# SimonMacLean/NeRF-or-nothing

Measured on AMD Instinct MI355X. Metric: train rays/sec (128 samples/ray, 8×256 MLP) at 1/2/4/8 MI355X; PSNR vs ref, higher is better.
Workload: dtype f32; 1 GPU; BASELINE configs[1]: 1024-ray global batch x 128+128 samples, 8x256 MLP fwd/bwd + Adam; global_batch=1024, rays_per_gpu=1024, micro_batch=1024, parallelism=dp1, precision=f32

## Files before the change

### nerf-or-nothing_amd/csrc/kernels/mlp16.h

```cpp
#pragma once
#include "mlp_common.h"

namespace nof {

constexpr int kMlp16Threads = 512;
constexpr int kIpe16Floats = 6 * 64 * 4;

__device__ __forceinline__ f32x4 mfma16(float a, float b, f32x4 c) {
  return __builtin_amdgcn_mfma_f32_16x16x4f32(a, b, c, 0, 0, 0);
}

__device__ __forceinline__ void slice16_dma_step(const float* __restrict__ src, float* dst, int tid, int i) {
  const int wave = tid >> 6;
  const __amdgpu_buffer_rsrc_t rsrc =
      __builtin_amdgcn_make_buffer_rsrc(const_cast<float*>(src), (short)0, 0x7fffffff, 0x00020000);
  __builtin_amdgcn_raw_ptr_buffer_load_lds(rsrc, (lptr_t)(dst + (kMlp16Threads * i + 64 * wave) * 4), 16, tid * 16,
                                           i * kMlp16Threads * 16, 0, 0);
}
__device__ __forceinline__ void slice16_dma(const float* __restrict__ src, float* dst, int tid) {
#pragma unroll
  for (int i = 0; i < 4; ++i) slice16_dma_step(src, dst, tid, i);
}

template <int P> constexpr int ring16_slots() { return P == 0 ? 4 : 3; }
template <int P> constexpr int ring16_floats() { return ring16_slots<P>() * kSliceFloats; }
__device__ __forceinline__ void ring16_prologue(const float* __restrict__ img, float* lds, int tid) {
  slice16_dma(img, lds, tid);
  slice16_dma(img + kSliceFloats, lds + kSliceFloats, tid);
}

__device__ __forceinline__ constexpr int feat16(int t, int g, int r) { return 16 * t + 4 * g + r; }

constexpr int kStoreNT = 2;
struct BlkStore16 {
  static constexpr bool kHalf = false;
  uint32_t voff[4];
  __device__ __forceinline__ BlkStore16(int lane, int half) {
    const int g = lane >> 4, s = 16 * half + (lane & 15);
#pragma unroll
    for (int r = 0; r < 4; ++r)
      voff[r] = 512u * g + ((((s >> 2) ^ (4 * (g & 1) + r)) << 4) | ((s & 3) << 2));
  }
  __device__ __forceinline__ void store(__amdgpu_buffer_rsrc_t blk, int t, int r, float v) const {
    __builtin_amdgcn_raw_buffer_store_b32(__float_as_uint(v), blk, (int)voff[r], 2048 * t + 128 * r, kStoreNT);
  }
};
__device__ __forceinline__ __amdgpu_buffer_rsrc_t blk_rsrc(float* blk) {
  return __builtin_amdgcn_make_buffer_rsrc(blk, (short)0, 0x7fffffff, 0x00020000);
}

template <bool kNT>
struct BlkStore16H {
  static constexpr bool kHalf = true;
  uint32_t voff;
  uint32_t voff2;
  uint32_t sel;
  __device__ __forceinline__ BlkStore16H(int lane, int half) {
    const int g = lane >> 4, j = lane & 15;
    voff = 256u * g + ((((2 * half + (j >> 3)) ^ g) << 4) | ((j & 7) << 1));
    voff2 = 256u * g + 64u * (j & 1) + ((((2 * half + (j >> 3)) ^ g) << 4) | ((j & 6) << 1));
    sel = (j & 1) ? 0x03020706u : 0x05040100u;
  }
  __device__ __forceinline__ void store_pairs(__amdgpu_buffer_rsrc_t blk, int t, uint32_t p01, uint32_t p23) const {
    const uint32_t q01 = (uint32_t)__builtin_amdgcn_mov_dpp((int)p01, 0xB1, 0xF, 0xF, false);
    const uint32_t q23 = (uint32_t)__builtin_amdgcn_mov_dpp((int)p23, 0xB1, 0xF, 0xF, false);
    __builtin_amdgcn_raw_buffer_store_b32(__builtin_amdgcn_perm(q01, p01, sel), blk, (int)voff2, 1024 * t,
                                          kNT ? kStoreNT : 0);
    __builtin_amdgcn_raw_buffer_store_b32(__builtin_amdgcn_perm(q23, p23, sel), blk, (int)voff2 + 128, 1024 * t,
                                          kNT ? kStoreNT : 0);
  }
  __device__ __forceinline__ void store(__amdgpu_buffer_rsrc_t blk, int t, int r, float v) const {
    store_h(blk, t, r, (_Float16)v);
  }
  __device__ __forceinline__ void store_h(__amdgpu_buffer_rsrc_t blk, int t, int r, _Float16 h) const {
    __builtin_amdgcn_raw_buffer_store_b16(__builtin_bit_cast(unsigned short, h), blk, (int)voff + 64 * r, 1024 * t,
                                          kNT ? kStoreNT : 0);
  }
};
template <int P, bool kBwd> struct Store16 { typedef BlkStore16 T; typedef float E; };
template <bool kBwd> struct Store16<2, kBwd> { typedef BlkStore16H<true> T; typedef _Float16 E; };
template <class E>
// ... 26 lines not shown
  typedef float f2 __attribute__((ext_vector_type(2)));
  hi01 = __builtin_bit_cast(uint32_t, __builtin_convertvector((f2{x[0], x[1]}), h2));
  hi23 = __builtin_bit_cast(uint32_t, __builtin_convertvector((f2{x[2], x[3]}), h2));
  float r[4];
  asm("v_fma_mix_f32 %0, %1, 1.0, -%2 op_sel_hi:[0,0,1]" : "=v"(r[0]) : "v"(x[0]), "v"(hi01));
  asm("v_fma_mix_f32 %0, %1, 1.0, -%2 op_sel:[0,0,1] op_sel_hi:[0,0,1]" : "=v"(r[1]) : "v"(x[1]), "v"(hi01));
  asm("v_fma_mix_f32 %0, %1, 1.0, -%2 op_sel_hi:[0,0,1]" : "=v"(r[2]) : "v"(x[2]), "v"(hi23));
  asm("v_fma_mix_f32 %0, %1, 1.0, -%2 op_sel:[0,0,1] op_sel_hi:[0,0,1]" : "=v"(r[3]) : "v"(x[3]), "v"(hi23));
  lo01 = __builtin_bit_cast(uint32_t, __builtin_convertvector((f2{r[0], r[1]}), h2));
  lo23 = __builtin_bit_cast(uint32_t, __builtin_convertvector((f2{r[2], r[3]}), h2));
}

template <bool kSplit, bool kStore, class ST>
__device__ __forceinline__ void put_tile(float (&bin)[16][4], int t, const float (&v)[4], const ST& bst,
                                         __amdgpu_buffer_rsrc_t blk) {
  if constexpr (kSplit) {
    uint32_t hi01, hi23, lo01, lo23;
    split4h(v, hi01, hi23, lo01, lo23);
    const int row = t & ~1, c = 2 * (t & 1);
    bin[row][c] = __uint_as_float(hi01);
    bin[row][c + 1] = __uint_as_float(hi23);
    bin[row + 1][c] = __uint_as_float(lo01);
    bin[row + 1][c + 1] = __uint_as_float(lo23);
    if constexpr (kStore) {
      if constexpr (ST::kHalf) {
        bst.store_pairs(blk, t, hi01, hi23);
      } else {
#pragma unroll
        for (int r = 0; r < 4; ++r) bst.store(blk, t, r, v[r]);
      }
    }
  } else {
#pragma unroll
    for (int r = 0; r < 4; ++r) {
      bin[t][r] = v[r];
      if constexpr (kStore) bst.store(blk, t, r, v[r]);
    }
  }
}

struct NoEpi16 {
  static constexpr int kVmPerPart = 0;
  __device__ __forceinline__ void operator()(int) {}
};

template <int NT_B, int NT_I, int OT, int kSlots, class Epi>
__device__ __forceinline__ void mlp_layer16(const float (&bin)[16][4], const float* ipe, f32x4 (&acc)[16],
                                            float* lds, int& cur, const float*& wsrc, bool last_in_schedule, int tid,
                                            int lane, Epi& epi, const float* cinit) {
  static_assert(OT % 2 == 0 && OT <= 16, "row tiles come in pairs");
  constexpr int NG = OT;
  constexpr int kEpiGroup1 = 4;
  constexpr int kEpiGroup2 = (NG / 2 + 4 < NG) ? NG / 2 + 4 : NG - 1;
  const int g = lane >> 4;
  const int row = lane & 15;
  const int swz = (row >> 1) & 7;
#pragma unroll
  for (int t = 0; t < NT_B + NT_I; ++t) {
    const bool dma = !(last_in_schedule && t + 2 >= NT_B + NT_I);
    const int nxt2 = kSlots == 4 ? ((cur + 2) & 3) : (cur == 0 ? 2 : cur - 1);
    const float* W = lds + cur * kSliceFloats + row * 32;
    auto aread = [&](int q, int which) {
      const int tt = q / (OT / 2), p = q % (OT / 2);
      return *reinterpret_cast<const f32x4*>(W + (2 * p + which) * 16 * 32 + (((4 * tt + g) ^ swz) << 2));
    };
    f32x4 a0 = aread(0, 0), a1 = aread(0, 1);
    auto cread = [&](int p, int which) { return *reinterpret_cast<const f32x4*>(cinit + 16 * (2 * p + which)); };
    f32x4 c0 = {}, c1 = {};
    if (t == 0 && cinit) { c0 = cread(0, 0); c1 = cread(0, 1); }
#pragma unroll
    for (int q = 0; q < NG; ++q) {
      const int tt = q / (OT / 2), p = q % (OT / 2);
      f32x4 b4;
      if (t < NT_B) {
        const int tb = (t < NT_B) ? 2 * t + tt : 0;
        b4[0] = bin[tb][0]; b4[1] = bin[tb][1]; b4[2] = bin[tb][2]; b4[3] = bin[tb][3];
      } else {
        const int ti = (t >= NT_B) ? 2 * (t - NT_B) + tt : 0;
        if constexpr (kSlots == 4) {
          b4[0] = ipe[4 * ti]; b4[1] = ipe[4 * ti + 1]; b4[2] = ipe[4 * ti + 2]; b4[3] = ipe[4 * ti + 3];
        } else b4 = *reinterpret_cast<const f32x4*>(ipe + (ti * 64 + lane) * 4);
      }
      asm volatile("" ::"v"(a0), "v"(a1), "v"(c0), "v"(c1));
      f32x4 n0 = a0, n1 = a1, m0 = c0, m1 = c1;
      if (q + 1 < NG) {
        n0 = aread(q + 1, 0);
        n1 = aread(q + 1, 1);
      }
      if (t == 0 && cinit && q + 1 < OT / 2) { m0 = cread(q + 1, 0); m1 = cread(q + 1, 1); }
      if (dma && q < 4) slice16_dma_step(wsrc + 2 * kSliceFloats, lds + nxt2 * kSliceFloats, tid, q);
      __builtin_amdgcn_sched_barrier(0);
      const bool first = t == 0 && tt == 0;
#pragma unroll
      for (int r = 0; r < 4; ++r) {
        acc[2 * p] = mfma16(a0[r], b4[r], (first && r == 0) ? c0 : acc[2 * p]);
        acc[2 * p + 1] = mfma16(a1[r], b4[r], (first && r == 0) ? c1 : acc[2 * p + 1]);
      }
      if (t + 1 < NT_B && q == kEpiGroup1) epi(2 * t + 2);
      if (t + 1 < NT_B && q == kEpiGroup2) epi(2 * t + 3);
      __builtin_amdgcn_sched_barrier(0);
      a0 = n0;
      a1 = n1;
      c0 = m0;
      c1 = m1;
    }
    if constexpr (kSlots == 4) {
      if (cur & 1) slice_barrier(t + 1 < NT_B ? 2 * Epi::kVmPerPart : 0);
      cur = (cur + 1) & 3;
    } else {
      slice_barrier((dma ? 4 : 0) + (t + 1 < NT_B ? 2 * Epi::kVmPerPart : 0));
      cur = cur == 2 ? 0 : cur + 1;
    }
    wsrc += kSliceFloats;
  }
}
template <int NT_B, int NT_I, int OT, class Epi>
__device__ __forceinline__ void mlp_layer16h(const float (&bin)[16][4], const float* ipe_lds, f32x4 (&acc)[16],
                                             float* lds, int& cur, const float*& wsrc, bool last_in_schedule, int tid,
                                             int lane, Epi& epi, const float* cinit) {
  typedef SplitMode<2> SM;
  static_assert(OT % 2 == 0 && OT <= 16, "row tiles come in pairs");
  constexpr int kPieces = 2;
  constexpr int kPP0 = 0;
  constexpr int kDmaSteps = 4;
  constexpr int kSlots = ring16_slots<2>();
  constexpr int NG = OT / 2;
  constexpr int kE1 = NG > 4 ? 4 : NG - 1;
  constexpr int kE2 = NG > 6 ? 6 : NG - 1;
#pragma unroll
  for (int t = 0; t < NT_B + NT_I; ++t) {
    const bool dma = !(last_in_schedule && t + 2 >= NT_B + NT_I);
    const int nxt2 = kSlots == 4 ? ((cur + 2) & 3) : (cur == 0 ? 2 : cur - 1);
    const f16x8* W = reinterpret_cast<const f16x8*>(lds + cur * kSliceFloats) + lane;
    Frag<2> b;
    float v[8];
    if (t < NT_B) {
      const int tb = t < NT_B ? 2 * t : 0;
      const f32x4 hi = {bin[tb][0], bin[tb][1], bin[tb][2], bin[tb][3]};
      const f32x4 lo = {bin[tb + 1][0], bin[tb + 1][1], bin[tb + 1][2], bin[tb + 1][3]};
      b.p[0] = __builtin_bit_cast(f16x8, hi);
      b.p[1] = __builtin_bit_cast(f16x8, lo);
    } else {
      const int ti = t >= NT_B ? 2 * (t - NT_B) : 0;
      if constexpr (kSlots == 4) {
#pragma unroll
        for (int i = 0; i < 8; ++i) v[i] = ipe_lds[4 * ti + i];
      } else {
        const f32x4 u0 = *reinterpret_cast<const f32x4*>(ipe_lds + (ti * 64 + lane) * 4);
        const f32x4 u1 = *reinterpret_cast<const f32x4*>(ipe_lds + ((ti + 1) * 64 + lane) * 4);
#pragma unroll
        for (int i = 0; i < 4; ++i) { v[i] = u0[i]; v[4 + i] = u1[i]; }
      }
      split8<2>(v, b);
    }
    Frag<2> a0, a1;
#pragma unroll
    for (int p = 0; p < kPieces; ++p) { a0.p[p] = W[(16 * p) * 64]; a1.p[p] = W[(16 * p + 1) * 64]; }
    auto cread = [&](int rt) { return *reinterpret_cast<const f32x4*>(cinit + 16 * rt); };
    f32x4 c0 = {}, c1 = {};
    if (t == 0 && cinit) { c0 = cread(0); c1 = cread(1); }
#pragma unroll
    for (int q = 0; q < NG; ++q) {
      if constexpr (kPieces == 2) asm volatile("" ::"v"(a0.p[0]), "v"(a0.p[1]), "v"(a1.p[0]), "v"(a1.p[1]), "v"(c0), "v"(c1));
      else asm volatile("" ::"v"(a0.p[0]), "v"(a1.p[0]), "v"(c0), "v"(c1));
      Frag<2> n0 = a0, n1 = a1;
      f32x4 m0 = c0, m1 = c1;
      if (t == 0 && cinit && q + 1 < NG) { m0 = cread(2 * q + 2); m1 = cread(2 * q + 3); }
      if (q + 1 < NG) {
#pragma unroll
        for (int p = 0; p < kPieces; ++p) {
          n0.p[p] = W[(16 * p + 2 * q + 2) * 64];
          n1.p[p] = W[(16 * p + 2 * q + 3) * 64];
        }
      }
      if (dma && q < kDmaSteps) slice16_dma_step(wsrc + 2 * kSliceFloats, lds + nxt2 * kSliceFloats, tid, q);
      __builtin_amdgcn_sched_barrier(0);
      const bool first = t == 0;
#pragma unroll
      for (int pp = kPP0; pp < SM::NPROD; ++pp) {
        acc[2 * q] = SM::mfma16(a0.p[SM::pa(pp)], b.p[SM::pb(pp)], (first && pp == kPP0) ? c0 : acc[2 * q]);
        acc[2 * q + 1] = SM::mfma16(a1.p[SM::pa(pp)], b.p[SM::pb(pp)], (first && pp == kPP0) ? c1 : acc[2 * q + 1]);
      }
      if (t + 1 < NT_B && q == kE1) epi(2 * t + 2);
      if (t + 1 < NT_B && q == kE2) epi(2 * t + 3);
      __builtin_amdgcn_sched_barrier(0);
      a0 = n0;
      a1 = n1;
      c0 = m0;
      c1 = m1;
    }
    if constexpr (kSlots == 4) {
      if (cur & 1) slice_barrier(t + 1 < NT_B ? 2 * Epi::kVmPerPart : 0);
      cur = (cur + 1) & 3;
    } else {
      slice_barrier((dma ? kDmaSteps : 0) + (t + 1 < NT_B ? 2 * Epi::kVmPerPart : 0));
      cur = cur == 2 ? 0 : cur + 1;
    }
    wsrc += kSliceFloats;
  }
}

template <int P, int NT_B, int NT_I, int OT, class Epi>
__device__ __forceinline__ void layer16(const float (&bin)[16][4], const float* ipe_lds, f32x4 (&acc)[16], float* lds,
                                        int& cur, const float*& wsrc, bool last_in_schedule, int tid, int lane,
                                        Epi& epi, const float* cinit = nullptr) {
  if constexpr (P == 2 || P == 3)
    mlp_layer16h<NT_B, NT_I, OT>(bin, ipe_lds, acc, lds, cur, wsrc, last_in_schedule, tid, lane, epi, cinit);
  else
    mlp_layer16<NT_B, NT_I, OT, ring16_slots<P>()>(bin, ipe_lds, acc, lds, cur, wsrc, last_in_schedule, tid, lane,
                                                   epi, cinit);
}
template <int P, int NT_B, int NT_I, int OT>
__device__ __forceinline__ void layer16(const float (&bin)[16][4], const float* ipe_lds, f32x4 (&acc)[16], float* lds,
                                        int& cur, const float*& wsrc, bool last_in_schedule, int tid, int lane,
                                        const float* cinit = nullptr) {
  NoEpi16 none;
  layer16<P, NT_B, NT_I, OT>(bin, ipe_lds, acc, lds, cur, wsrc, last_in_schedule, tid, lane, none, cinit);
}

}
```

### nerf-or-nothing_amd/csrc/kernels/mlp_bwd16.hip

```cpp
#include "common.h"
#include "launch.h"
#include "mlp16.h"

namespace nof {


template <bool kDensity, class ST, bool kSplit = false>
struct BwdEpi16 {
  static constexpr int kVmPerPart = 4;
  const f32x4 (&acc)[16];
  float (&bin)[16][4];
  const ST& bst;
  const int g;
  const float* w8;
  float dzs;
  __amdgpu_buffer_rsrc_t dst_blk;
  uint2 mk;
  f32x4 wnext;

  __device__ __forceinline__ BwdEpi16(const f32x4 (&acc_)[16], float (&bin_)[16][4], const ST& bst_, int lane)
      : acc(acc_), bin(bin_), bst(bst_), g(lane >> 4) {}
  template <class E>
  __device__ __forceinline__ void begin(const uint2* mask, E* dst_blk_, const float* w8_ = nullptr, float dzs_ = 0.0f) {
    mk = *mask;
    dst_blk = blk_rsrc_t(dst_blk_);
    if constexpr (kDensity) {
      w8 = w8_ + 4 * g;
      dzs = dzs_;
      wnext = *reinterpret_cast<const f32x4*>(w8);
    }
  }
  __device__ __forceinline__ void operator()(int t) {
    f32x4 w4;
    if constexpr (kDensity) {
      w4 = wnext;
      if (t + 1 < 16) wnext = *reinterpret_cast<const f32x4*>(w8 + 16 * (t + 1));
    }
    float v[4];
#pragma unroll
    for (int r = 0; r < 4; ++r) {
      v[r] = acc[t][r];
      if constexpr (kDensity) v[r] = __builtin_fmaf(w4[r], dzs, v[r]);
      v[r] = mask16_apply(mk, t, r, v[r]);
    }
    put_tile<kSplit, true>(bin, t, v, bst, dst_blk);
  }
  __device__ __forceinline__ void tile01() {
    (*this)(0);
    (*this)(1);
  }
};

template <int P>
__global__ __launch_bounds__(kMlp16Threads, 1) void k_mlp_bwd16(BwdArgs a) {
  typedef typename Store16<P, true>::T ST;
  typedef typename Store16<P, true>::E AE;
  __shared__ __attribute__((aligned(16))) float lds[ring16_floats<P>() + 256];
  float* w8_lds = lds + ring16_floats<P>();
  const int tid = threadIdx.x, lane = tid & 63, g = lane >> 4, j = lane & 15;
  const int wave = __builtin_amdgcn_readfirstlane(tid >> 6);
  const int half = wave & 1;
  const ST bst(lane, half);
  const int nblk = a.M / kBlk;
  const int blk_raw = blockIdx.x * 4 + (wave >> 1);
  const int blk = blk_raw < nblk ? blk_raw : nblk - 1;
  const int m = blk * kBlk + 16 * half + j;
  NOF_DCHECK(a.M % kBlk == 0 && blk >= 0 && blk < nblk, kChkMlpBlock);
  const float* tail = a.wimg_b + (size_t)kBwdSlices * kSliceFloats;
  const size_t layer_stride = (size_t)nblk * kWidth * kBlk;
  uint32_t* masks = const_cast<uint32_t*>(a.masks);

  ring16_prologue(a.wimg_b, lds, tid);

  const f32x4 zh = reinterpret_cast<const f32x4*>(a.zhead)[m];
  float dzs = a.dsigma[m] * sigmoid_f(zh[0] + a.dbias);
  float dzc[3];
#pragma unroll
  for (int c = 0; c < 3; ++c) {
    const float s = sigmoid_f(zh[1 + c]);
    dzc[c] = a.drgb[(size_t)m * 3 + c] * (s * (1.0f - s)) * a.rgb_scale;
  }
  if constexpr (P >= 2) {
    const float sc = delta_scale(a.amax, false);
    dzs *= sc;
#pragma unroll
    for (int c = 0; c < 3; ++c) dzc[c] *= sc;
  }
  const __amdgpu_buffer_rsrc_t d9 = blk_rsrc_t(reinterpret_cast<AE*>(a.delta9x) + (size_t)blk * kD9F * kBlk);
#pragma unroll
  for (int r = 0; r < 4; ++r) bst.store(d9, 8, r, g == 0 ? (r == 0 ? dzs : dzc[r - 1]) : 0.0f);
  float bin[16][4];
  {
    const uint2 mk = *mask16_ptr(masks, blk, 8, half, lane);
    const float* w10 = tail + kBwdTailW10;
#pragma unroll
    for (int t = 0; t < 8; ++t) {
      const int fb = 16 * t + 4 * g;
      const f32x4 wa = *reinterpret_cast<const f32x4*>(w10 + fb);
      const f32x4 wb = *reinterpret_cast<const f32x4*>(w10 + 128 + fb);
      const f32x4 wc = *reinterpret_cast<const f32x4*>(w10 + 256 + fb);
      float v[4];
#pragma unroll
      for (int r = 0; r < 4; ++r)
        v[r] = mask16_apply(mk, t, r, __builtin_fmaf(wc[r], dzc[2], __builtin_fmaf(wb[r], dzc[1], wa[r] * dzc[0])));
      put_tile<P >= 2, true>(bin, t, v, bst, d9);
    }
  }
  if (tid < 64) reinterpret_cast<f32x4*>(w8_lds)[tid] = reinterpret_cast<const f32x4*>(tail + kBwdTailW8)[tid];
  __syncthreads();

  int cur = 0;
  const float* wsrc = a.wimg_b;
  f32x4 accA[16], accB[16];
  AE* delta_blk = reinterpret_cast<AE*>(a.delta) + (size_t)blk * kWidth * kBlk;
  BwdEpi16<true, ST, P >= 2> e7(accA, bin, bst, lane);
  e7.begin(mask16_ptr(masks, blk, 7, half, lane), delta_blk + 7 * layer_stride, w8_lds, dzs);
  layer16<P, 4, 0, 16>(bin, nullptr, accA, lds, cur, wsrc, false, tid, lane);
  e7.tile01();
  BwdEpi16<false, ST, P >= 2> ea(accA, bin, bst, lane), eb(accB, bin, bst, lane);
  eb.begin(mask16_ptr(masks, blk, 6, half, lane), delta_blk + 6 * layer_stride);
  layer16<P, 8, 0, 16>(bin, nullptr, accB, lds, cur, wsrc, false, tid, lane, e7);
  eb.tile01();
  static_assert(kDepth == 8, "bwd pairing assumes 8 trunk layers");
  for (int l = kDepth - 2; l >= 2; l -= 2) {
    ea.begin(mask16_ptr(masks, blk, l - 1, half, lane), delta_blk + (l - 1) * layer_stride);
    layer16<P, 8, 0, 16>(bin, nullptr, accA, lds, cur, wsrc, false, tid, lane, eb);
    ea.tile01();
    eb.begin(mask16_ptr(masks, blk, l - 2, half, lane), delta_blk + (l - 2) * layer_stride);
    layer16<P, 8, 0, 16>(bin, nullptr, accB, lds, cur, wsrc, l == 2, tid, lane, ea);
    eb.tile01();
  }
#pragma unroll
  for (int t = 2; t < 16; ++t) eb(t);
}

hipError_t launch_mlp_bwd16(const BwdArgs& a, hipStream_t st) {
  const int nblk = a.M / kBlk;
  if (a.split == 2) hipLaunchKernelGGL(k_mlp_bwd16<2>, dim3((nblk + 3) / 4), dim3(kMlp16Threads), 0, st, a);
  else if (a.split == 3) hipLaunchKernelGGL(k_mlp_bwd16<3>, dim3((nblk + 3) / 4), dim3(kMlp16Threads), 0, st, a);
  else hipLaunchKernelGGL(k_mlp_bwd16<0>, dim3((nblk + 3) / 4), dim3(kMlp16Threads), 0, st, a);
  return hipGetLastError();
}

NOF_CHECK_UNIT(check_unit_mlp_bwd16)

}
```

### nerf-or-nothing_amd/csrc/kernels/mlp_fwd16.hip

```cpp
#include "common.h"
#include "geometry.h"
#include "launch.h"
#include "mlp16.h"

namespace nof {


template <bool store, bool kDensity, int NT, class ST, bool kSplit = false>
struct FwdEpi16 {
  static constexpr int kVmPerPart = store ? 4 : 0;
  const f32x4 (&acc)[16];
  float (&bin)[16][4];
  const ST& bst;
  const int g;
  const float* w8;
  __amdgpu_buffer_rsrc_t act_blk;
  uint2* mask_dst;
  uint32_t mw[2];
  f32x4 wnext;
  float zs;

  __device__ __forceinline__ FwdEpi16(const f32x4 (&acc_)[16], float (&bin_)[16][4], const ST& bst_, int lane)
      : acc(acc_), bin(bin_), bst(bst_), g(lane >> 4) {}
  template <class E>
  __device__ __forceinline__ void begin(E* act_blk_, uint2* mask_dst_, const float* w8_ = nullptr) {
    act_blk = blk_rsrc_t(act_blk_);
    mask_dst = mask_dst_;
    mw[0] = mw[1] = 0u;
    if constexpr (kDensity) {
      w8 = w8_ + 4 * g;
      wnext = *reinterpret_cast<const f32x4*>(w8);
      zs = 0.0f;
    }
  }
  __device__ __forceinline__ void operator()(int t) {
    const bool more = t + 1 < NT;
    f32x4 w4;
    if constexpr (kDensity) {
      w4 = wnext;
      if (more) wnext = *reinterpret_cast<const f32x4*>(w8 + 16 * (t + 1));
    }
    float hv[4];
#pragma unroll
    for (int r = 0; r < 4; ++r) {
      hv[r] = relu_bit(acc[t][r], mw[t >> 3]);
      if constexpr (kDensity) zs = __builtin_fmaf(w4[r], hv[r], zs);
    }
    put_tile<kSplit, store>(bin, t, hv, bst, act_blk);
    if constexpr (store && kVmPerPart > 0)
      if (!more) *mask_dst = make_uint2(mw[0], mw[1]);
  }
  __device__ __forceinline__ void tile01() {
    (*this)(0);
    (*this)(1);
  }
};

template <int P, bool store>
__global__ __launch_bounds__(kMlp16Threads, 1) void k_mlp_fwd16(FwdArgs a) {
  typedef typename Store16<P, false>::T ST;
  typedef typename Store16<P, false>::E AE;
  constexpr int kRing = ring16_slots<P>() * kSliceFloats;
  constexpr bool kIpeReg = ring16_slots<P>() == 4;
  constexpr int kIpeLds = kIpeReg ? 0 : 8 * kIpe16Floats;
  constexpr int kBiasLds = 8 * 256 + 256;
  __shared__ __attribute__((aligned(16))) float lds[kRing + kIpeLds + 8 * 128 + kBiasLds];
  const int tid = threadIdx.x, lane = tid & 63, g = lane >> 4, j = lane & 15;
  const int wave = __builtin_amdgcn_readfirstlane(tid >> 6);
  const int half = wave & 1;
  const int nblk = a.M / kBlk;
  const int blk_raw = blockIdx.x * 4 + (wave >> 1);
  const int blk = blk_raw < nblk ? blk_raw : nblk - 1;
  const int m0 = blk * kBlk;
  const int ray = m0 / a.S;
  const int s0 = m0 - ray * a.S + 16 * half;
  const int m = m0 + 16 * half + j;
  const float* tail = a.wimg + (size_t)kFwdSlices * kSliceFloats;
  NOF_DCHECK(a.M % kBlk == 0 && a.S % kBlk == 0 && blk >= 0 && blk < nblk, kChkMlpBlock);

  ring16_prologue(a.wimg, lds, tid);

  float ipe[6][4];
  float d3[3];
  if (!a.encoded) {
    d3[0] = a.dirs[3 * ray]; d3[1] = a.dirs[3 * ray + 1]; d3[2] = a.dirs[3 * ray + 2];
    const float o3[3] = {a.origins[3 * ray], a.origins[3 * ray + 1], a.origins[3 * ray + 2]};
    const float* tr = a.t + (size_t)ray * (a.S + 1) + s0 + j;
    float mean[3], cov[3];
    frustum_gaussian(tr[0], tr[1], o3, d3, a.radii[ray], mean, cov, a.cylinder != 0);
#pragma unroll
    for (int t = 0; t < 6; ++t)
#pragma unroll
      for (int r = 0; r < 4; ++r)
        ipe[t][r] = ipe_feature(feat16(t, g, r), mean, cov);
  } else {
#pragma unroll
    for (int t = 0; t < 6; ++t)
#pragma unroll
      for (int r = 0; r < 4; ++r) ipe[t][r] = a.enc_pos[(size_t)m * kPosIn + feat16(t, g, r)];
  }
  const int kl = lane < kDirIn ? lane : 0;
  const float pe_l = a.encoded ? a.enc_dir[(size_t)ray * kDirIn + kl] : dir_feature(kl, d3);
  float pe[kDirIn];
#pragma unroll
  for (int k = 0; k < kDirIn; ++k) pe[k] = __int_as_float(__builtin_amdgcn_readlane(__float_as_int(pe_l), k));

  const ST bst(lane, half);
  if constexpr (store) {
    const __amdgpu_buffer_rsrc_t act_in_rs = blk_rsrc_t(reinterpret_cast<AE*>(a.act_in) + (size_t)blk * kInF * kBlk);
#pragma unroll
    for (int t = 0; t < 6; ++t)
#pragma unroll
      for (int r = 0; r < 4; ++r) bst.store(act_in_rs, t, r, ipe[t][r]);
#pragma unroll
    for (int t = 6; t < 8; ++t)
#pragma unroll
      for (int r = 0; r < 4; ++r) {
        const int k = feat16(t, g, r) - kPosIn;
        float v = 0.0f;
#pragma unroll
        for (int kk = 0; kk < kDirIn; ++kk) v = (kk == k) ? pe[kk] : v;
        bst.store(act_in_rs, t, r, v);
      }
  }
  const float* ipe_b = &ipe[0][0];
  if constexpr (!kIpeReg) {
    float* ipe_lds = lds + kRing + wave * kIpe16Floats;
#pragma unroll
    for (int t = 0; t < 6; ++t) {
      f32x4 v;
      v[0] = ipe[t][0]; v[1] = ipe[t][1]; v[2] = ipe[t][2]; v[3] = ipe[t][3];
      *reinterpret_cast<f32x4*>(ipe_lds + (t * 64 + lane) * 4) = v;
    }
    ipe_b = ipe_lds;
  }
  float* dirb = lds + kRing + kIpeLds + wave * 128;
  float* bias_lds = lds + kRing + kIpeLds + 8 * 128;
  for (int i = tid; i < kBiasLds / 4; i += kMlp16Threads) {
    const float* src = i < 512 ? tail + kFwdTailBias + 4 * i : tail + kFwdTailW8 + 4 * (i - 512);
    *reinterpret_cast<f32x4*>(bias_lds + 4 * i) = *reinterpret_cast<const f32x4*>(src);
  }
#pragma unroll
  for (int rep = 0; rep < 2; ++rep) {
    const int o = lane + 64 * rep;
    float s = tail[kFwdTailBias + 9 * 256 + o];
    const float* w9 = tail + kFwdTailW9d + o * 32;
#pragma unroll
    for (int k = 0; k < kDirIn; ++k) s = __builtin_fmaf(w9[k], pe[k], s);
    dirb[o] = s;
  }
  __syncthreads();

  int cur = 0;
  const float* wsrc = a.wimg;
  f32x4 accA[16], accB[16];
  float bin[16][4];
  const size_t layer_stride = (size_t)nblk * kWidth * kBlk;
  const float* biases = bias_lds;
  AE* act_h_blk = reinterpret_cast<AE*>(a.act_h) + (size_t)blk * kWidth * kBlk;

  constexpr bool kPre = P >= 2;
  FwdEpi16<store, false, 16, ST, kPre> ea(accA, bin, bst, lane), eb(accB, bin, bst, lane);
  const float* bias_g = biases + 4 * g;
  ea.begin(act_h_blk, mask16_ptr(a.masks, blk, 0, half, lane));
  layer16<P, 0, 3, 16>(bin, ipe_b, accA, lds, cur, wsrc, false, tid, lane, bias_g);
  ea.tile01();
  for (int l = 1; l < kDepth - 1; l += 2) {
    eb.begin(act_h_blk + l * layer_stride, mask16_ptr(a.masks, blk, l, half, lane));
    layer16<P, 8, 0, 16>(bin, ipe_b, accB, lds, cur, wsrc, false, tid, lane, ea, bias_g + l * 256);
    eb.tile01();
    ea.begin(act_h_blk + (l + 1) * layer_stride, mask16_ptr(a.masks, blk, l + 1, half, lane));
    if (l + 1 == kSkip)
      layer16<P, 8, 3, 16>(bin, ipe_b, accA, lds, cur, wsrc, false, tid, lane, eb, bias_g + (l + 1) * 256);
    else layer16<P, 8, 0, 16>(bin, ipe_b, accA, lds, cur, wsrc, false, tid, lane, eb, bias_g + (l + 1) * 256);
    ea.tile01();
  }
  static_assert(kDepth == 8 && kSkip % 2 == 0, "trunk pairing assumes 8 layers and an even skip layer");
  FwdEpi16<store, true, 16, ST, kPre> e7(accB, bin, bst, lane);
  e7.begin(act_h_blk + 7 * layer_stride, mask16_ptr(a.masks, blk, 7, half, lane), bias_lds + 8 * 256);
  layer16<P, 8, 0, 16>(bin, ipe_b, accB, lds, cur, wsrc, false, tid, lane, ea, bias_g + 7 * 256);
  e7.tile01();

  layer16<P, 8, 0, 8>(bin, ipe_b, accA, lds, cur, wsrc, true, tid, lane, e7, dirb + 4 * g);
  float zs = e7.zs;
  zs += __shfl_xor(zs, 16, 64);
  zs += __shfl_xor(zs, 32, 64);
  zs += tail[kFwdTailBias + 8 * 256];
  FwdEpi16<store, false, 8, ST> e9(accA, bin, bst, lane);
  e9.begin(reinterpret_cast<AE*>(a.act_h9) + (size_t)blk * kWidthCond * kBlk, mask16_ptr(a.masks, blk, 8, half, lane));
#pragma unroll
  for (int t = 0; t < 8; ++t) e9(t);

  float zc[3] = {0.0f, 0.0f, 0.0f};
#pragma unroll
  for (int c = 0; c < 3; ++c) {
#pragma unroll
    for (int t = 0; t < 8; ++t) {
      const f32x4 w4 = *reinterpret_cast<const f32x4*>(tail + kFwdTailW10 + c * 128 + 16 * t + 4 * g);
#pragma unroll
      for (int r = 0; r < 4; ++r) zc[c] = __builtin_fmaf(w4[r], bin[t][r], zc[c]);
    }
    zc[c] += __shfl_xor(zc[c], 16, 64);
    zc[c] += __shfl_xor(zc[c], 32, 64);
    zc[c] += tail[kFwdTailBias + 10 * 256 + c];
  }

  if (g == 0) {
    a.sigma[m] = softplus_f(zs + a.dbias);
#pragma unroll
    for (int c = 0; c < 3; ++c) a.rgb[(size_t)m * 3 + c] = sigmoid_f(zc[c]) * a.rgb_scale - a.rgb_pad;
    f32x4 zh;
    zh[0] = zs; zh[1] = zc[0]; zh[2] = zc[1]; zh[3] = zc[2];
    if constexpr (store) reinterpret_cast<f32x4*>(a.zhead)[m] = zh;
  }
}

hipError_t launch_mlp_fwd16(const FwdArgs& a, hipStream_t st) {
  const int nblk = a.M / kBlk;
  const dim3 grid((nblk + 3) / 4), block(kMlp16Threads);
  if (a.split == 2) {
    if (a.no_store) hipLaunchKernelGGL((k_mlp_fwd16<2, false>), grid, block, 0, st, a);
    else hipLaunchKernelGGL((k_mlp_fwd16<2, true>), grid, block, 0, st, a);
  } else if (a.split == 3) {
    if (a.no_store) hipLaunchKernelGGL((k_mlp_fwd16<2, false>), grid, block, 0, st, a);
    else hipLaunchKernelGGL((k_mlp_fwd16<3, true>), grid, block, 0, st, a);
  } else {
    if (a.no_store) hipLaunchKernelGGL((k_mlp_fwd16<0, false>), grid, block, 0, st, a);
    else hipLaunchKernelGGL((k_mlp_fwd16<0, true>), grid, block, 0, st, a);
  }
  return hipGetLastError();
}

NOF_CHECK_UNIT(check_unit_mlp_fwd16)

}
```

### nerf-or-nothing_amd/csrc/kernels/stamps.h

```cpp
#pragma once
#include "common.h"

namespace nof {
#ifdef NOF_WG_STAMPS
__device__ unsigned long long g_wg_times[2][1024][2];
#define NOF_WG_T0(k) const unsigned long long wg_t0_ = wall_clock64();
#define NOF_WG_T1(k)                                                                   \
  __syncthreads();                                                                     \
  if (threadIdx.x == 0 && blockIdx.x < 1024) {                                         \
    g_wg_times[k][blockIdx.x][0] = wg_t0_;                                             \
    g_wg_times[k][blockIdx.x][1] = wall_clock64();                                     \
  }
__device__ unsigned long long g_item_times[2][4096][4];
#define NOF_IT_T0(k) const unsigned long long it_t0_ = wall_clock64();
#define NOF_IT_T1(k)                                                                 \
  if (threadIdx.x == 0 && it < 4096) {                                               \
    g_item_times[k][it][0] = it_t0_;                                                 \
    g_item_times[k][it][1] = wall_clock64();                                         \
    g_item_times[k][it][2] = item.prob | (blockIdx.x << 16);                         \
    g_item_times[k][it][3] = item.kb1 - item.kb0;                                    \
  }
extern "C" int nof_diag_item_times(unsigned long long* host, int kernel) {
  return (int)hipMemcpyFromSymbol(host, HIP_SYMBOL(g_item_times), sizeof(unsigned long long) * 16384,
                                  sizeof(unsigned long long) * 16384 * kernel, hipMemcpyDeviceToHost);
}
extern "C" int nof_diag_wg_times(unsigned long long* host, int kernel) {
  return (int)hipMemcpyFromSymbol(host, HIP_SYMBOL(g_wg_times), sizeof(unsigned long long) * 2048,
                                  sizeof(unsigned long long) * 2048 * kernel, hipMemcpyDeviceToHost);
}
#else
#define NOF_WG_T0(k)
#define NOF_WG_T1(k)
#define NOF_IT_T0(k)
#define NOF_IT_T1(k)
#endif

}
```

### nerf-or-nothing_amd/csrc/kernels/wgrad.hip

```cpp
#include "common.h"
#include "launch.h"
#include "mlp_common.h"
#include "stamps.h"

namespace nof {

constexpr int kWgThreads = 512;
__host__ __device__ constexpr int wg_piece_off(int g) { return g * 8 * kBlk + 64 * (g >> 2) + 32 * ((g >> 1) & 1); }
constexpr int kWgHalf = wg_piece_off(32);
__device__ __forceinline__ int wg_row_off(int row) { return wg_piece_off(row >> 3) + (row & 7) * kBlk; }

typedef __attribute__((address_space(3))) void* wg_lptr_t;

struct WgShape { int gc, rb, cb, rot; };
constexpr WgShape kWgShapes[] = {{4, 4, 2, 1}, {1, 1, 3, 1}, {1, 1, 1, 1}, {8, 5, 1, 1}, {8, 1, 1, 1}, {4, 4, 2, 0}};
constexpr int kWgNumShapes = sizeof(kWgShapes) / sizeof(kWgShapes[0]);

template <int GC, int RB, int CB, bool ROT>
__device__ __forceinline__ void wg_item(const WgItem& item, const WgProblem& P, float* lds, int tid, int lane,
                                        int wave, float* slabs, float* bias_slabs, const int64_t* slab_off) {
  const int h = lane >> 5, x = lane & 31;
  const int wr = wave / GC, wc = wave % GC;
  const int r0 = wr * RB, c0 = wc * CB;
  const bool active = r0 < P.ntr && c0 < P.ntc;
  int rowt[RB], colt[CB];
#pragma unroll
  for (int r = 0; r < RB; ++r) rowt[r] = min(r0 + (ROT ? (r + wc) % RB : r), P.ntr - 1);
#pragma unroll
  for (int c = 0; c < CB; ++c) colt[c] = min(c0 + c, P.ntc - 1);
  const float* Ab = P.A + (size_t)P.a_row0 * kBlk;
  const float* Bb = P.B + (size_t)P.b_col0 * kBlk;
  const size_t strideA = (size_t)P.FA * kBlk, strideB = (size_t)P.FB * kBlk;

  f32x16 acc[RB][CB];
  f32x2 bs[ROT ? 1 : RB];
#pragma unroll
  for (int r = 0; r < (ROT ? 1 : RB); ++r) bs[r] = f32x2{0.0f, 0.0f};
#pragma unroll
  for (int r = 0; r < RB; ++r) {
#pragma unroll
    for (int c = 0; c < CB; ++c)
#pragma unroll
      for (int e = 0; e < 16; ++e) acc[r][c][e] = 0.0f;
  }
  int aoff[RB], boff[CB];
#pragma unroll
  for (int r = 0; r < RB; ++r) aoff[r] = wg_row_off(rowt[r] * 32 + x);
#pragma unroll
  for (int c = 0; c < CB; ++c) boff[c] = wg_row_off(colt[c] * 32 + x);
  const int xs = x & 7;

  constexpr int NJ = ((8 / GC) * RB + GC * CB + 1) / 2;
  const int npA = P.ntr * 4, npT = npA + P.ntc * 4;
  const int wv = __builtin_amdgcn_readfirstlane(wave);
  auto dma_step = [&](int kbn, float* buf, int j) {
// ... 913 lines not shown
```

Measured before the change: 161,800 rays/s.

## Run f32 MLP forward with 256-thread workgroups, two per CU, double-buffered weight ring

For the f32 (P==0) forward kernel, the workgroup shrinks from 512 to 256 threads with launch bounds allowing two workgroups per CU. The LDS weight ring drops from four slots to two, prefetching one slice ahead with per-slice barriers. The goal is more independent workgroups per CU, so barrier and DMA stalls in one can be hidden by the other, and finer grid granularity. The cost is a shallower prefetch that may expose weight-load latency, more DMA steps per thread, and register pressure. The backward kernel is templated the same way but still uses 512 threads, and optional timing stamps are added.

```diff
diff --git a/nerf-or-nothing_amd/csrc/kernels/mlp16.h b/nerf-or-nothing_amd/csrc/kernels/mlp16.h
--- a/nerf-or-nothing_amd/csrc/kernels/mlp16.h
+++ b/nerf-or-nothing_amd/csrc/kernels/mlp16.h
@@ -3,30 +3,35 @@
 
 namespace nof {
 
-constexpr int kMlp16Threads = 512;
+template <int P, bool kBwd> constexpr int mlp16_threads() { return P == 0 && !kBwd ? 256 : 512; }
+template <int kT> constexpr int mlp16_wg_per_cu() { return kT == 256 ? 2 : 1; }
 constexpr int kIpe16Floats = 6 * 64 * 4;
 
 __device__ __forceinline__ f32x4 mfma16(float a, float b, f32x4 c) {
   return __builtin_amdgcn_mfma_f32_16x16x4f32(a, b, c, 0, 0, 0);
 }
 
+template <int kThreads> constexpr int slice16_dma_steps() { return kSliceFloats / 4 / kThreads; }
+template <int kThreads = 512>
 __device__ __forceinline__ void slice16_dma_step(const float* __restrict__ src, float* dst, int tid, int i) {
   const int wave = tid >> 6;
   const __amdgpu_buffer_rsrc_t rsrc =
       __builtin_amdgcn_make_buffer_rsrc(const_cast<float*>(src), (short)0, 0x7fffffff, 0x00020000);
-  __builtin_amdgcn_raw_ptr_buffer_load_lds(rsrc, (lptr_t)(dst + (kMlp16Threads * i + 64 * wave) * 4), 16, tid * 16,
-                                           i * kMlp16Threads * 16, 0, 0);
-}
+  __builtin_amdgcn_raw_ptr_buffer_load_lds(rsrc, (lptr_t)(dst + (kThreads * i + 64 * wave) * 4), 16, tid * 16,
+                                           i * kThreads * 16, 0, 0);
+}
+template <int kThreads>
 __device__ __forceinline__ void slice16_dma(const float* __restrict__ src, float* dst, int tid) {
 #pragma unroll
-  for (int i = 0; i < 4; ++i) slice16_dma_step(src, dst, tid, i);
-}
-
-template <int P> constexpr int ring16_slots() { return P == 0 ? 4 : 3; }
-template <int P> constexpr int ring16_floats() { return ring16_slots<P>() * kSliceFloats; }
+  for (int i = 0; i < slice16_dma_steps<kThreads>(); ++i) slice16_dma_step<kThreads>(src, dst, tid, i);
+}
+
+template <int P, int kT> constexpr int ring16_slots() { return P != 0 ? 3 : kT == 256 ? 2 : 4; }
+template <int P, int kT> constexpr int ring16_floats() { return ring16_slots<P, kT>() * kSliceFloats; }
+template <int P, int kT>
 __device__ __forceinline__ void ring16_prologue(const float* __restrict__ img, float* lds, int tid) {
-  slice16_dma(img, lds, tid);
-  slice16_dma(img + kSliceFloats, lds + kSliceFloats, tid);
+  slice16_dma<kT>(img, lds, tid);
+  if constexpr (ring16_slots<P, kT>() > 2) slice16_dma<kT>(img + kSliceFloats, lds + kSliceFloats, tid);
 }
 
 __device__ __forceinline__ constexpr int feat16(int t, int g, int r) { return 16 * t + 4 * g + r; }
@@ -159,13 +164,18 @@
   constexpr int NG = OT;
   constexpr int kEpiGroup1 = 4;
   constexpr int kEpiGroup2 = (NG / 2 + 4 < NG) ? NG / 2 + 4 : NG - 1;
+  constexpr int kThreads = kSlots == 2 ? 256 : 512;
+  constexpr int kSteps = slice16_dma_steps<kThreads>();
+  constexpr int kAhead = kSlots == 2 ? 1 : 2;
+  constexpr int kPartsAfterDma = (kEpiGroup1 >= kSteps - 1) + (kEpiGroup2 >= kSteps - 1);
+  static_assert(NG >= kSteps, "one DMA step per MFMA group");
   const int g = lane >> 4;
   const int row = lane & 15;
   const int swz = (row >> 1) & 7;
 #pragma unroll
   for (int t = 0; t < NT_B + NT_I; ++t) {
-    const bool dma = !(last_in_schedule && t + 2 >= NT_B + NT_I);
-    const int nxt2 = kSlots == 4 ? ((cur + 2) & 3) : (cur == 0 ? 2 : cur - 1);
+    const bool dma = !(last_in_schedule && t + kAhead >= NT_B + NT_I);
+    const int nxt2 = kSlots == 2 ? (cur ^ 1) : kSlots == 4 ? ((cur + 2) & 3) : (cur == 0 ? 2 : cur - 1);
     const float* W = lds + cur * kSliceFloats + row * 32;
     auto aread = [&](int q, int which) {
       const int tt = q / (OT / 2), p = q % (OT / 2);
@@ -184,7 +194,7 @@
         b4[0] = bin[tb][0]; b4[1] = bin[tb][1]; b4[2] = bin[tb][2]; b4[3] = bin[tb][3];
       } else {
         const int ti = (t >= NT_B) ? 2 * (t - NT_B) + tt : 0;
-        if constexpr (kSlots == 4) {
+        if constexpr (kSlots != 3) {
           b4[0] = ipe[4 * ti]; b4[1] = ipe[4 * ti + 1]; b4[2] = ipe[4 * ti + 2]; b4[3] = ipe[4 * ti + 3];
         } else b4 = *reinterpret_cast<const f32x4*>(ipe + (ti * 64 + lane) * 4);
       }
@@ -195,7 +205,8 @@
         n1 = aread(q + 1, 1);
       }
       if (t == 0 && cinit && q + 1 < OT / 2) { m0 = cread(q + 1, 0); m1 = cread(q + 1, 1); }
-      if (dma && q < 4) slice16_dma_step(wsrc + 2 * kSliceFloats, lds + nxt2 * kSliceFloats, tid, q);
+      if (dma && q < kSteps)
+        slice16_dma_step<kThreads>(wsrc + kAhead * kSliceFloats, lds + nxt2 * kSliceFloats, tid, q);
       __builtin_amdgcn_sched_barrier(0);
       const bool first = t == 0 && tt == 0;
 #pragma unroll
@@ -211,11 +222,14 @@
       c0 = m0;
       c1 = m1;
     }
-    if constexpr (kSlots == 4) {
-      if (cur & 1) slice_barrier(t + 1 < NT_B ? 2 * Epi::kVmPerPart : 0);
+    if constexpr (kSlots == 2) {
+      if (dma) slice_barrier(t + 1 < NT_B ? kPartsAfterDma * Epi::kVmPerPart : 0);
+      cur ^= 1;
+    } else if constexpr (kSlots == 4) {
+      if (cur & 1) slice_barrier(t + 1 < NT_B ? kPartsAfterDma * Epi::kVmPerPart : 0);
       cur = (cur + 1) & 3;
     } else {
-      slice_barrier((dma ? 4 : 0) + (t + 1 < NT_B ? 2 * Epi::kVmPerPart : 0));
+      slice_barrier((dma ? kSteps : 0) + (t + 1 < NT_B ? 2 * Epi::kVmPerPart : 0));
       cur = cur == 2 ? 0 : cur + 1;
     }
     wsrc += kSliceFloats;
@@ -230,7 +244,7 @@
   constexpr int kPieces = 2;
   constexpr int kPP0 = 0;
   constexpr int kDmaSteps = 4;
-  constexpr int kSlots = ring16_slots<2>();
+  constexpr int kSlots = ring16_slots<2, 512>();
   constexpr int NG = OT / 2;
   constexpr int kE1 = NG > 4 ? 4 : NG - 1;
   constexpr int kE2 = NG > 6 ? 6 : NG - 1;
@@ -280,7 +294,7 @@
           n1.p[p] = W[(16 * p + 2 * q + 3) * 64];
         }
       }
-      if (dma && q < kDmaSteps) slice16_dma_step(wsrc + 2 * kSliceFloats, lds + nxt2 * kSliceFloats, tid, q);
+      if (dma && q < kDmaSteps) slice16_dma_step<512>(wsrc + 2 * kSliceFloats, lds + nxt2 * kSliceFloats, tid, q);
       __builtin_amdgcn_sched_barrier(0);
       const bool first = t == 0;
 #pragma unroll
@@ -307,22 +321,23 @@
   }
 }
 
-template <int P, int NT_B, int NT_I, int OT, class Epi>
+template <int P, int kT, int NT_B, int NT_I, int OT, class Epi>
 __device__ __forceinline__ void layer16(const float (&bin)[16][4], const float* ipe_lds, f32x4 (&acc)[16], float* lds,
                                         int& cur, const float*& wsrc, bool last_in_schedule, int tid, int lane,
                                         Epi& epi, const float* cinit = nullptr) {
-  if constexpr (P == 2 || P == 3)
+  if constexpr (P == 2 || P == 3) {
+    static_assert(kT == 512, "the f16 layers stream by 512 threads");
     mlp_layer16h<NT_B, NT_I, OT>(bin, ipe_lds, acc, lds, cur, wsrc, last_in_schedule, tid, lane, epi, cinit);
-  else
-    mlp_layer16<NT_B, NT_I, OT, ring16_slots<P>()>(bin, ipe_lds, acc, lds, cur, wsrc, last_in_schedule, tid, lane,
+  } else
+    mlp_layer16<NT_B, NT_I, OT, ring16_slots<P, kT>()>(bin, ipe_lds, acc, lds, cur, wsrc, last_in_schedule, tid, lane,
                                                    epi, cinit);
 }
-template <int P, int NT_B, int NT_I, int OT>
+template <int P, int kT, int NT_B, int NT_I, int OT>
 __device__ __forceinline__ void layer16(const float (&bin)[16][4], const float* ipe_lds, f32x4 (&acc)[16], float* lds,
                                         int& cur, const float*& wsrc, bool last_in_schedule, int tid, int lane,
                                         const float* cinit = nullptr) {
   NoEpi16 none;
-  layer16<P, NT_B, NT_I, OT>(bin, ipe_lds, acc, lds, cur, wsrc, last_in_schedule, tid, lane, none, cinit);
-}
-
-}
+  layer16<P, kT, NT_B, NT_I, OT>(bin, ipe_lds, acc, lds, cur, wsrc, last_in_schedule, tid, lane, none, cinit);
+}
+
+}
diff --git a/nerf-or-nothing_amd/csrc/kernels/mlp_bwd16.hip b/nerf-or-nothing_amd/csrc/kernels/mlp_bwd16.hip
--- a/nerf-or-nothing_amd/csrc/kernels/mlp_bwd16.hip
+++ b/nerf-or-nothing_amd/csrc/kernels/mlp_bwd16.hip
@@ -1,9 +1,11 @@
 #include "common.h"
 #include "launch.h"
 #include "mlp16.h"
+#include "stamps.h"
 
 namespace nof {
 
+NOF_MLP_STAMPS(bwd)
 
 template <bool kDensity, class ST, bool kSplit = false>
 struct BwdEpi16 {
@@ -52,25 +54,29 @@
 };
 
 template <int P>
-__global__ __launch_bounds__(kMlp16Threads, 1) void k_mlp_bwd16(BwdArgs a) {
+__global__ __launch_bounds__((mlp16_threads<P, true>()), (mlp16_wg_per_cu<mlp16_threads<P, true>()>()))
+void k_mlp_bwd16(BwdArgs a) {
+  constexpr int kThreads = mlp16_threads<P, true>(), kWaves = kThreads / 64;
   typedef typename Store16<P, true>::T ST;
   typedef typename Store16<P, true>::E AE;
-  __shared__ __attribute__((aligned(16))) float lds[ring16_floats<P>() + 256];
-  float* w8_lds = lds + ring16_floats<P>();
+  __shared__ __attribute__((aligned(16))) float lds[ring16_floats<P, kThreads>() + 256];
+  static_assert(mlp16_wg_per_cu<kThreads>() * sizeof(lds) <= 160 * 1024, "LDS per CU");
+  float* w8_lds = lds + ring16_floats<P, kThreads>();
   const int tid = threadIdx.x, lane = tid & 63, g = lane >> 4, j = lane & 15;
   const int wave = __builtin_amdgcn_readfirstlane(tid >> 6);
   const int half = wave & 1;
   const ST bst(lane, half);
   const int nblk = a.M / kBlk;
-  const int blk_raw = blockIdx.x * 4 + (wave >> 1);
+  const int blk_raw = blockIdx.x * (kWaves / 2) + (wave >> 1);
   const int blk = blk_raw < nblk ? blk_raw : nblk - 1;
   const int m = blk * kBlk + 16 * half + j;
   NOF_DCHECK(a.M % kBlk == 0 && blk >= 0 && blk < nblk, kChkMlpBlock);
   const float* tail = a.wimg_b + (size_t)kBwdSlices * kSliceFloats;
   const size_t layer_stride = (size_t)nblk * kWidth * kBlk;
   uint32_t* masks = const_cast<uint32_t*>(a.masks);
+  NOF_MLP_T(0)
 
-  ring16_prologue(a.wimg_b, lds, tid);
+  ring16_prologue<P, kThreads>(a.wimg_b, lds, tid);
 
   const f32x4 zh = reinterpret_cast<const f32x4*>(a.zhead)[m];
   float dzs = a.dsigma[m] * sigmoid_f(zh[0] + a.dbias);
@@ -108,6 +114,7 @@
   }
   if (tid < 64) reinterpret_cast<f32x4*>(w8_lds)[tid] = reinterpret_cast<const f32x4*>(tail + kBwdTailW8)[tid];
   __syncthreads();
+  NOF_MLP_T(1)
 
   int cur = 0;
   const float* wsrc = a.wimg_b;
@@ -115,30 +122,34 @@
   AE* delta_blk = reinterpret_cast<AE*>(a.delta) + (size_t)blk * kWidth * kBlk;
   BwdEpi16<true, ST, P >= 2> e7(accA, bin, bst, lane);
   e7.begin(mask16_ptr(masks, blk, 7, half, lane), delta_blk + 7 * layer_stride, w8_lds, dzs);
-  layer16<P, 4, 0, 16>(bin, nullptr, accA, lds, cur, wsrc, false, tid, lane);
+  layer16<P, kThreads, 4, 0, 16>(bin, nullptr, accA, lds, cur, wsrc, false, tid, lane);
   e7.tile01();
   BwdEpi16<false, ST, P >= 2> ea(accA, bin, bst, lane), eb(accB, bin, bst, lane);
   eb.begin(mask16_ptr(masks, blk, 6, half, lane), delta_blk + 6 * layer_stride);
-  layer16<P, 8, 0, 16>(bin, nullptr, accB, lds, cur, wsrc, false, tid, lane, e7);
+  layer16<P, kThreads, 8, 0, 16>(bin, nullptr, accB, lds, cur, wsrc, false, tid, lane, e7);
   eb.tile01();
   static_assert(kDepth == 8, "bwd pairing assumes 8 trunk layers");
   for (int l = kDepth - 2; l >= 2; l -= 2) {
     ea.begin(mask16_ptr(masks, blk, l - 1, half, lane), delta_blk + (l - 1) * layer_stride);
-    layer16<P, 8, 0, 16>(bin, nullptr, accA, lds, cur, wsrc, false, tid, lane, eb);
+    layer16<P, kThreads, 8, 0, 16>(bin, nullptr, accA, lds, cur, wsrc, false, tid, lane, eb);
     ea.tile01();
     eb.begin(mask16_ptr(masks, blk, l - 2, half, lane), delta_blk + (l - 2) * layer_stride);
-    layer16<P, 8, 0, 16>(bin, nullptr, accB, lds, cur, wsrc, l == 2, tid, lane, ea);
+    layer16<P, kThreads, 8, 0, 16>(bin, nullptr, accB, lds, cur, wsrc, l == 2, tid, lane, ea);
     eb.tile01();
   }
+  NOF_MLP_T(2)
 #pragma unroll
   for (int t = 2; t < 16; ++t) eb(t);
+  if constexpr (P == 0) { NOF_MLP_TEND(bwd) }
 }
 
 hipError_t launch_mlp_bwd16(const BwdArgs& a, hipStream_t st) {
   const int nblk = a.M / kBlk;
-  if (a.split == 2) hipLaunchKernelGGL(k_mlp_bwd16<2>, dim3((nblk + 3) / 4), dim3(kMlp16Threads), 0, st, a);
-  else if (a.split == 3) hipLaunchKernelGGL(k_mlp_bwd16<3>, dim3((nblk + 3) / 4), dim3(kMlp16Threads), 0, st, a);
-  else hipLaunchKernelGGL(k_mlp_bwd16<0>, dim3((nblk + 3) / 4), dim3(kMlp16Threads), 0, st, a);
+  static_assert(mlp16_threads<2, true>() == 512 && mlp16_threads<3, true>() == 512, "grids below");
+  constexpr int kT0 = mlp16_threads<0, true>(), kPer0 = kT0 / 128;
+  if (a.split == 2) hipLaunchKernelGGL(k_mlp_bwd16<2>, dim3((nblk + 3) / 4), dim3(512), 0, st, a);
+  else if (a.split == 3) hipLaunchKernelGGL(k_mlp_bwd16<3>, dim3((nblk + 3) / 4), dim3(512), 0, st, a);
+  else hipLaunchKernelGGL(k_mlp_bwd16<0>, dim3((nblk + kPer0 - 1) / kPer0), dim3(kT0), 0, st, a);
   return hipGetLastError();
 }
 
diff --git a/nerf-or-nothing_amd/csrc/kernels/mlp_fwd16.hip b/nerf-or-nothing_amd/csrc/kernels/mlp_fwd16.hip
--- a/nerf-or-nothing_amd/csrc/kernels/mlp_fwd16.hip
+++ b/nerf-or-nothing_amd/csrc/kernels/mlp_fwd16.hip
@@ -2,9 +2,11 @@
 #include "geometry.h"
 #include "launch.h"
 #include "mlp16.h"
+#include "stamps.h"
 
 namespace nof {
 
+NOF_MLP_STAMPS(fwd)
 
 template <bool store, bool kDensity, int NT, class ST, bool kSplit = false>
 struct FwdEpi16 {
@@ -57,19 +59,22 @@
 };
 
 template <int P, bool store>
-__global__ __launch_bounds__(kMlp16Threads, 1) void k_mlp_fwd16(FwdArgs a) {
+__global__ __launch_bounds__((mlp16_threads<P, false>()), (mlp16_wg_per_cu<mlp16_threads<P, false>()>()))
+void k_mlp_fwd16(FwdArgs a) {
+  constexpr int kThreads = mlp16_threads<P, false>(), kWaves = kThreads / 64;
   typedef typename Store16<P, false>::T ST;
   typedef typename Store16<P, false>::E AE;
-  constexpr int kRing = ring16_slots<P>() * kSliceFloats;
-  constexpr bool kIpeReg = ring16_slots<P>() == 4;
-  constexpr int kIpeLds = kIpeReg ? 0 : 8 * kIpe16Floats;
+  constexpr int kRing = ring16_floats<P, kThreads>();
+  constexpr bool kIpeReg = P == 0;
+  constexpr int kIpeLds = kIpeReg ? 0 : kWaves * kIpe16Floats;
   constexpr int kBiasLds = 8 * 256 + 256;
-  __shared__ __attribute__((aligned(16))) float lds[kRing + kIpeLds + 8 * 128 + kBiasLds];
+  __shared__ __attribute__((aligned(16))) float lds[kRing + kIpeLds + kWaves * 128 + kBiasLds];
+  static_assert(mlp16_wg_per_cu<kThreads>() * sizeof(lds) <= 160 * 1024, "LDS per CU");
   const int tid = threadIdx.x, lane = tid & 63, g = lane >> 4, j = lane & 15;
   const int wave = __builtin_amdgcn_readfirstlane(tid >> 6);
   const int half = wave & 1;
   const int nblk = a.M / kBlk;
-  const int blk_raw = blockIdx.x * 4 + (wave >> 1);
+  const int blk_raw = blockIdx.x * (kWaves / 2) + (wave >> 1);
   const int blk = blk_raw < nblk ? blk_raw : nblk - 1;
   const int m0 = blk * kBlk;
   const int ray = m0 / a.S;
@@ -77,8 +82,9 @@
   const int m = m0 + 16 * half + j;
   const float* tail = a.wimg + (size_t)kFwdSlices * kSliceFloats;
   NOF_DCHECK(a.M % kBlk == 0 && a.S % kBlk == 0 && blk >= 0 && blk < nblk, kChkMlpBlock);
-
-  ring16_prologue(a.wimg, lds, tid);
+  NOF_MLP_T(0)
+
+  ring16_prologue<P, kThreads>(a.wimg, lds, tid);
 
   float ipe[6][4];
   float d3[3];
@@ -135,8 +141,8 @@
     ipe_b = ipe_lds;
   }
   float* dirb = lds + kRing + kIpeLds + wave * 128;
-  float* bias_lds = lds + kRing + kIpeLds + 8 * 128;
-  for (int i = tid; i < kBiasLds / 4; i += kMlp16Threads) {
+  float* bias_lds = lds + kRing + kIpeLds + kWaves * 128;
+  for (int i = tid; i < kBiasLds / 4; i += kThreads) {
     const float* src = i < 512 ? tail + kFwdTailBias + 4 * i : tail + kFwdTailW8 + 4 * (i - 512);
     *reinterpret_cast<f32x4*>(bias_lds + 4 * i) = *reinterpret_cast<const f32x4*>(src);
   }
@@ -150,6 +156,7 @@
     dirb[o] = s;
   }
   __syncthreads();
+  NOF_MLP_T(1)
 
   int cur = 0;
   const float* wsrc = a.wimg;
@@ -163,25 +170,26 @@
   FwdEpi16<store, false, 16, ST, kPre> ea(accA, bin, bst, lane), eb(accB, bin, bst, lane);
   const float* bias_g = biases + 4 * g;
   ea.begin(act_h_blk, mask16_ptr(a.masks, blk, 0, half, lane));
-  layer16<P, 0, 3, 16>(bin, ipe_b, accA, lds, cur, wsrc, false, tid, lane, bias_g);
+  layer16<P, kThreads, 0, 3, 16>(bin, ipe_b, accA, lds, cur, wsrc, false, tid, lane, bias_g);
   ea.tile01();
   for (int l = 1; l < kDepth - 1; l += 2) {
     eb.begin(act_h_blk + l * layer_stride, mask16_ptr(a.masks, blk, l, half, lane));
-    layer16<P, 8, 0, 16>(bin, ipe_b, accB, lds, cur, wsrc, false, tid, lane, ea, bias_g + l * 256);
+    layer16<P, kThreads, 8, 0, 16>(bin, ipe_b, accB, lds, cur, wsrc, false, tid, lane, ea, bias_g + l * 256);
     eb.tile01();
     ea.begin(act_h_blk + (l + 1) * layer_stride, mask16_ptr(a.masks, blk, l + 1, half, lane));
     if (l + 1 == kSkip)
-      layer16<P, 8, 3, 16>(bin, ipe_b, accA, lds, cur, wsrc, false, tid, lane, eb, bias_g + (l + 1) * 256);
-    else layer16<P, 8, 0, 16>(bin, ipe_b, accA, lds, cur, wsrc, false, tid, lane, eb, bias_g + (l + 1) * 256);
+      layer16<P, kThreads, 8, 3, 16>(bin, ipe_b, accA, lds, cur, wsrc, false, tid, lane, eb, bias_g + (l + 1) * 256);
+    else layer16<P, kThreads, 8, 0, 16>(bin, ipe_b, accA, lds, cur, wsrc, false, tid, lane, eb, bias_g + (l + 1) * 256);
     ea.tile01();
   }
   static_assert(kDepth == 8 && kSkip % 2 == 0, "trunk pairing assumes 8 layers and an even skip layer");
   FwdEpi16<store, true, 16, ST, kPre> e7(accB, bin, bst, lane);
   e7.begin(act_h_blk + 7 * layer_stride, mask16_ptr(a.masks, blk, 7, half, lane), bias_lds + 8 * 256);
-  layer16<P, 8, 0, 16>(bin, ipe_b, accB, lds, cur, wsrc, false, tid, lane, ea, bias_g + 7 * 256);
+  layer16<P, kThreads, 8, 0, 16>(bin, ipe_b, accB, lds, cur, wsrc, false, tid, lane, ea, bias_g + 7 * 256);
   e7.tile01();
 
-  layer16<P, 8, 0, 8>(bin, ipe_b, accA, lds, cur, wsrc, true, tid, lane, e7, dirb + 4 * g);
+  layer16<P, kThreads, 8, 0, 8>(bin, ipe_b, accA, lds, cur, wsrc, true, tid, lane, e7, dirb + 4 * g);
+  NOF_MLP_T(2)
   float zs = e7.zs;
   zs += __shfl_xor(zs, 16, 64);
   zs += __shfl_xor(zs, 32, 64);
@@ -213,11 +221,15 @@
     zh[0] = zs; zh[1] = zc[0]; zh[2] = zc[1]; zh[3] = zc[2];
     if constexpr (store) reinterpret_cast<f32x4*>(a.zhead)[m] = zh;
   }
+  if constexpr (P == 0) { NOF_MLP_TEND(fwd) }
 }
 
 hipError_t launch_mlp_fwd16(const FwdArgs& a, hipStream_t st) {
   const int nblk = a.M / kBlk;
-  const dim3 grid((nblk + 3) / 4), block(kMlp16Threads);
+  const dim3 grid((nblk + 3) / 4), block(mlp16_threads<2, false>());
+  const dim3 grid0((nblk + 1) / 2), block0(mlp16_threads<0, false>());
+  static_assert(mlp16_threads<2, false>() == 512 && mlp16_threads<3, false>() == 512 &&
+                mlp16_threads<0, false>() == 256, "grids above");
   if (a.split == 2) {
     if (a.no_store) hipLaunchKernelGGL((k_mlp_fwd16<2, false>), grid, block, 0, st, a);
     else hipLaunchKernelGGL((k_mlp_fwd16<2, true>), grid, block, 0, st, a);
@@ -225,8 +237,8 @@
     if (a.no_store) hipLaunchKernelGGL((k_mlp_fwd16<2, false>), grid, block, 0, st, a);
     else hipLaunchKernelGGL((k_mlp_fwd16<3, true>), grid, block, 0, st, a);
   } else {
-    if (a.no_store) hipLaunchKernelGGL((k_mlp_fwd16<0, false>), grid, block, 0, st, a);
-    else hipLaunchKernelGGL((k_mlp_fwd16<0, true>), grid, block, 0, st, a);
+    if (a.no_store) hipLaunchKernelGGL((k_mlp_fwd16<0, false>), grid0, block0, 0, st, a);
+    else hipLaunchKernelGGL((k_mlp_fwd16<0, true>), grid0, block0, 0, st, a);
   }
   return hipGetLastError();
 }
diff --git a/nerf-or-nothing_amd/csrc/kernels/stamps.h b/nerf-or-nothing_amd/csrc/kernels/stamps.h
--- a/nerf-or-nothing_amd/csrc/kernels/stamps.h
+++ b/nerf-or-nothing_amd/csrc/kernels/stamps.h
@@ -3,6 +3,28 @@
 
 namespace nof {
 #ifdef NOF_WG_STAMPS
+constexpr int kMlpStampWgs = 4096;
+#define NOF_MLP_STAMPS(name)                                                                        \
+  __device__ unsigned long long g_mlp_times_##name[kMlpStampWgs][4];                                \
+  extern "C" int nof_diag_mlp_times_##name(unsigned long long* host) {                              \
+    return (int)hipMemcpyFromSymbol(host, HIP_SYMBOL(g_mlp_times_##name),                           \
+                                    sizeof(unsigned long long) * kMlpStampWgs * 4, 0, hipMemcpyDeviceToHost); \
+  }
+#define NOF_MLP_T(i) const unsigned long long mlp_t##i##_ = wall_clock64();
+#define NOF_MLP_TEND(name)                                              \
+  __syncthreads();                                                      \
+  if (threadIdx.x == 0 && blockIdx.x < kMlpStampWgs) {                  \
+    g_mlp_times_##name[blockIdx.x][0] = mlp_t0_;                        \
+    g_mlp_times_##name[blockIdx.x][1] = mlp_t1_;                        \
+    g_mlp_times_##name[blockIdx.x][2] = mlp_t2_;                        \
+    g_mlp_times_##name[blockIdx.x][3] = wall_clock64();                 \
+  }
+#else
+#define NOF_MLP_STAMPS(name)
+#define NOF_MLP_T(i)
+#define NOF_MLP_TEND(name)
+#endif
+#if defined(NOF_WG_STAMPS) && defined(NOF_STAMPS_WGRAD)
 __device__ unsigned long long g_wg_times[2][1024][2];
 #define NOF_WG_T0(k) const unsigned long long wg_t0_ = wall_clock64();
 #define NOF_WG_T1(k)                                                                   \
diff --git a/nerf-or-nothing_amd/csrc/kernels/wgrad.hip b/nerf-or-nothing_amd/csrc/kernels/wgrad.hip
--- a/nerf-or-nothing_amd/csrc/kernels/wgrad.hip
+++ b/nerf-or-nothing_amd/csrc/kernels/wgrad.hip
@@ -1,6 +1,7 @@
 #include "common.h"
 #include "launch.h"
 #include "mlp_common.h"
+#define NOF_STAMPS_WGRAD
 #include "stamps.h"
 
 namespace nof {
```

Measured after the change: 162,300 rays/s, median of 6. No clear change (+0.4%).
